# regeirk/pycwt

Measured on NVIDIA H100. Metric: cwt_scale_points_per_sec, higher is better.
Workload: dtype f64

## Files before the change

### pycwt_b200/csrc/engine.cu

```cuda
#include <algorithm>
#include <array>
#include <cmath>
#include <cstdint>
#include <cstdio>
#include <cstdlib>
#include <cstring>
#include <map>
#include <mutex>
#include <set>
#include <string>
#include <type_traits>
#include <vector>

#include <cuda_runtime.h>
#ifndef CWTB_HOST_EMU
#include <dlfcn.h>
#endif

#include "../../include/cwt_b200.h"
#include "kernels.cuh"

using namespace cwtb;

template <class B, class = void> struct BodyNT { static constexpr int value = NT; };
// ... 101 lines not shown
  unsigned n = 0, L = 0;
  double2 *wm = nullptr;
  double2 *bf[2] = {nullptr, nullptr};
};

struct NTabDev {
  double2 *hi = nullptr, *lo = nullptr;
  int h = 0;
};

struct cwtb_ctx {
  int device = 0;
  rt_stream stream{};
  rt_stream aux_stream{};
  rt_stream prio_stream{};
  rt_stream prio_aux[7]{};
  int prio_fan = 4;
  int prio_mode = 1;
  rt_stream chain_streams[3]{};
  int n_chains = 2;
  rt_stream cur{};
  int pad_pow2 = 1;
  int coh_precision = 0;
  std::map<unsigned, BluePlan> blue;
  long long serial = 0;
  int two_streams = 1;
  int three_streams = 1;
  rt_stream copy_streams[4]{};
  int d2h_split = 1;
  std::string err;
  double band_eps = 1e-16;
  double band_eps32 = 1e-9;
  double expand_eps = 5e-13;
  double expand_eps32 = 2e-7;
  int expand_mma = 1;
  int dense_margin = 2;
  int expand_min_log2R = 0;
  int os_on = 1;
  Buf osH, osgrp;
  Buf *ztmp = nullptr;
  void *comm = nullptr;
  int comm_world = 1, comm_rank = 0;
  Buf comm_send, comm_recv;
  int group = 0;
  size_t group_bytes = (size_t)512 << 20;
  size_t rows_chunk_bytes = (size_t)256 << 20;
  int l2_persist = 0;
  int direct_max_log2 = 13;
  int fused = 0;
  int ring = 3;
  int pipe_ahead = 2;
  int num_sms = 132;
  int pf_dist = 132;
  int gauss_rec = 1;
  int pf_rows_a = 32, pf_rows_b = 32;
  int pf_dist_a = 132;
  int k2_512_max_log2 = 16;
  int passb_rev = 1;
  int k2_band_log2 = 9;
  size_t batch_bytes = (size_t)4 << 30;
  double2 *tw64 = nullptr;
  float2 *tw32 = nullptr;
  std::map<unsigned, NTabDev> ntabs;
  Buf filt;
  int filt_rows = 0;
  long long filt_n = 0;
  Buf Zxs[7];
  Buf Zx, Cin, Cout, wtab;
  std::map<std::array<long long, 3>, long long> wtab_index;
  std::vector<double> wtab_host;
  size_t wtab_uploaded = 0;
  size_t wtab_max_bytes = (size_t)256 << 20;
  Buf ctr, sig, sig2, spec, Z, Zc[3], Y, B, W, W2, descs, table, scratch, C, A12, F, aux, rowd, win, mask, hist, noise, wide, blueA, blueX, blueY;
  Job job;
  struct PlanKey {
    long long n0 = -1;
    double dt = 0, param = 0, band_eps = 0, band_eps32 = 0, expand_eps = 0, expand_eps32 = 0;
    int S = 0, family = 0, precision = 0, nbatch = 0, pad = 0;
    std::vector<double> scales;
    bool operator==(const PlanKey &o) const {
      return n0 == o.n0 && dt == o.dt && param == o.param && band_eps == o.band_eps && band_eps32 == o.band_eps32 &&
             expand_eps == o.expand_eps && expand_eps32 == o.expand_eps32 && S == o.S && family == o.family &&
             precision == o.precision && nbatch == o.nbatch && pad == o.pad && scales == o.scales;
// ... 12 lines not shown
  const void *job_dsig = nullptr;
  double last_ms = 0;
  int launches = 0;
  std::set<const void *> configured;
  bool profiling = false;
  int prof_saved_streams = 1;
  const char *prof_tag = "";
  struct ProfRec { std::string name; unsigned gx, gy; int ev; };
  std::vector<ProfRec> prof;
#ifndef CWTB_HOST_EMU
  std::vector<cudaEvent_t> prof_events;
#endif
  std::set<void *> pinned, devallocs;
#ifndef CWTB_HOST_EMU
  cudaEvent_t e0{}, e1{};
  cudaEvent_t ev_fork{}, ev_join{}, ev_joinc[3]{}, ev_coarse{};
  cudaEvent_t ev_h2d[2]{}, ev_used[2]{};
  cudaEvent_t ev_xband{}, ev_pj[7]{}, ev_angle{};
#endif
};

static int fail(cwtb_ctx *c, int code, const std::string &msg);
static void apply_l2_policy(cwtb_ctx *c);
static int fail(cwtb_ctx *c, int code, const std::string &msg) {
  if (c) c->err = msg;
  return code;
}
#define RT(call)                                                                             \
  do {                                                                                       \
    int e_ = (call);                                                                         \
    if (e_ != 0) return fail(c, CWTB_ERR_CUDA, std::string(#call) + ": " + rt_errstr(e_));   \
  } while (0)

// ... 353 lines not shown
    if (xeps > 0 && !job.exact && family != CWTB_TABLE && khi >= klo && job.log2N >= 9 && band_limited) {
      const long long kc = (klo + khi) / 2 - (((klo + khi) % 2 != 0 && (klo + khi) < 0) ? 1 : 0);
      const long long hw = std::max(khi - kc, kc - klo);
#ifdef CWTB_HOST_EMU
      const bool mma = false;
      const int max_taps = precision == CWTB_F64 ? 20 : 10;
#else
      const bool mma = precision == CWTB_F64 && c->expand_mma && job.log2N >= 12;
      const int max_taps = mma ? 20 : (precision == CWTB_F64 ? 16 : 10);
#endif
      const long long need = max_taps > 16 ? (32 * hw + 10) / 11 : 4 * hw;
      int lmin = std::max(6, ilog2((unsigned long long)std::max<long long>(need, 1)));
      lmin = std::max(lmin, job.log2N - 14);
      double best = 1e300;
      const int min_log2R = c->expand_min_log2R ? c->expand_min_log2R : (mma ? 2 : 3);
      for (int l = lmin; l <= lmin + 2 && job.log2N - l >= min_log2R; ++l) {
        double xi_b = 0;
        int w = expand_taps((double)hw / (double)(1ll << l), xeps, precision != CWTB_F64, max_taps, &xi_b);
        if (!w) continue;
        if (mma) w = (w + 3) / 4 * 4;
        if (xi_b > 0.25 && expand_gain(fam, s, klo, khi, kc, l, w, M_PI * w * (1.0 - xi_b)) > 64.0) continue;
        const int ksteps = job.log2N - l == 2 ? (w + 4) / 4 : (w + 3) / 4;
        const double xcost = mma ? std::max(2.72, 0.83 * ksteps) : 0.06 * (2 * w + 8);
        const double cost = xcost + (mma ? 18.0 : 12.0) * (double)(1ll << l) / (double)N;
        if (cost < best) {
          best = cost;
          d.ip_log2Nc = l; d.ip_kc = (int)kc; d.ip_w = w;
          d.ip_beta = M_PI * w * (1.0 - xi_b);
          d.ip_dc = std::cyl_bessel_i(0.0, d.ip_beta) / w;
        }
      }
// ... 106 lines not shown
    case 10: return launch_passA<T, SIGN, 1024, MODE>(c, a, ny);
  }
  return fail(c, CWTB_ERR_UNSUPPORTED, "transform longer than 2^20 per row is not supported yet");
}

template <typename T, int SIGN>
static int two_kernel_rows(cwtb_ctx *c, const void *in, int real_in, long long in_pitch, long long n_in,
                           cx<T> *out, long long out_pitch, unsigned n, int nrows, long long nout,
                           const double *grow, double post, int ileave, const ScaleDesc *descs, int first,
                           int out_row0, int epi) {
  const int l2 = ilog2(n);
  NTab nt;
  int e = get_ntab(c, n, l2, &nt);
  if (e) return e;
  const int chunk = std::max(1, std::min(nrows, (int)std::max<size_t>(1, c->rows_chunk_bytes / ((size_t)n * sizeof(cx<T>)))));
  Buf &Zt = c->ztmp ? *c->ztmp : c->Z;
  if ((e = ensure(c, Zt, (size_t)chunk * n * sizeof(cx<T>)))) return e;
  for (int r0 = 0; r0 < nrows; r0 += chunk) {
    const int nr = std::min(chunk, nrows - r0);
    PassAArgs<T> a{};
    a.in = in; a.Z = (cx<T> *)Zt.p; a.tw = Tw<T>::get(c); a.nt = nt;
    a.in_pitch = in_pitch; a.n_in = n_in; a.N = n; a.first = 0; a.zmod = 1 << 30; a.K2 = K2C;
    a.row0 = (ileave > 1 ? 0 : out_row0) + r0;
    a.pf_dist = c->pf_rows_a;
    e = real_in ? dispatch_passA<T, SIGN, MODE_REAL>(c, l2 - 10, a, nr)
                : dispatch_passA<T, SIGN, MODE_CPLX>(c, l2 - 10, a, nr);
    if (e) return e;
    PassBArgs<T> b{};
    b.Z = (const cx<T> *)Zt.p; b.out = out; b.tw = Tw<T>::get(c); b.descs = descs;
    b.pitch = out_pitch; b.nout = nout; b.N = n; b.first = first;
    b.epi = grow ? EPI_GAUSS : epi; b.grow = grow; b.post = post; b.zmod = 1 << 30;
// ... 496 lines not shown
      cudaEvent_t e;
      RT(cudaEventCreate(&e));
      c->prof_events.push_back(e);
    }
    c->prof.push_back({std::string(c->prof_tag) + body_name(__PRETTY_FUNCTION__), grid, rows, ev});
    RT(cudaEventRecord(c->prof_events[ev], c->cur));
  }
  kern<<<grid, Body::NTB, Body::SMEM, c->cur>>>(a, gm, (unsigned)total);
  RT(cudaGetLastError());
  if (ev >= 0) RT(cudaEventRecord(c->prof_events[ev + 1], c->cur));
  c->launches++;
  return 0;
}
#endif

template <typename T, int TAPS>
static int launch_expand_t(cwtb_ctx *c, const ExpandArgs<T> &a, int rows, int min_log2Nc) {
  using B = ExpandBody<T, TAPS>;
  const unsigned gx = std::max<unsigned>(1, a.N / (unsigned)(B::NT * B::L));
#ifndef CWTB_HOST_EMU
  if constexpr (std::is_same<T, double>::value) {
    static_assert(ExpandMmaBody<TAPS>::OUT_PER_CTA == 4096, "the planner assumes the tensor-core kernel from Np = 2^12");
    if (c->expand_mma && a.N >= (unsigned)ExpandMmaBody<TAPS>::OUT_PER_CTA) {
      const unsigned gm = a.N / (32u * std::min<unsigned>(ExpandMmaBody<TAPS>::L, 1u << min_log2Nc));
      if (a.epi == EPI_MULCONJ) return launch_persistent<ExpandMmaBody<TAPS, EPI_MULCONJ>>(c, gm, rows, a);
      return launch_persistent<ExpandMmaBody<TAPS>>(c, gm, rows, a);
    }
  }
#endif
#ifndef CWTB_HOST_EMU
// ... 24 lines not shown
    }
  }
  return fail(c, CWTB_ERR_STATE, "expansion: unsupported tap count");
}

template <typename T>
static int run_job(cwtb_ctx *c, const Job &job, const T *dsig, cx<T> *Wout = nullptr, int epi = EPI_STORE) {
  using V = cx<T>;
  if (job.exact) {
    if constexpr (std::is_same<T, double>::value) return run_job_exact(c, job, dsig, Wout, epi);
    else return fail(c, CWTB_ERR_UNSUPPORTED, "un-padded transforms run in fp64");
  }
  const unsigned N = job.N;
  const int S = job.S * job.nbatch;
  int e;
  struct CurGuard { cwtb_ctx *c; ~CurGuard() { c->cur = c->stream; c->prof_tag = ""; c->ztmp = nullptr; } } cur_guard{c};
  if ((e = ensure(c, c->spec, (size_t)job.nbatch * N * sizeof(V)))) return e;
  if (!Wout) {
    if ((e = ensure(c, c->W, (size_t)S * job.n0 * sizeof(V)))) return e;
    Wout = (V *)c->W.p;
  }
  V *spec = (V *)c->spec.p;
  V *W = Wout;
  const ScaleDesc *ddesc = (const ScaleDesc *)c->descs.p;
  Fam fam = job.fam;
  if (fam.family == CWTB_TABLE) fam.table = (const double2 *)c->table.p;

  if (N < 32) {
    if (job.nbatch != 1) return fail(c, CWTB_ERR_UNSUPPORTED, "batched transform needs n0 > 16");
    TinyFwdArgs<T> fa{dsig, spec, job.n0, N};
    if ((e = launch<TinyFwdBody<T>>(c, 1, 1, fa))) return e;
// ... 28 lines not shown
    }
  }
  const bool split = c->two_streams != 0;
#ifndef CWTB_HOST_EMU
  const bool split2 = split && c->three_streams && !c->fused;
  if (split) {
    RT(cudaEventRecord(c->ev_fork, c->stream));
    RT(cudaStreamWaitEvent(c->aux_stream, c->ev_fork, 0));
    if (split2)
      for (int k = 1; k < c->n_chains; ++k) RT(cudaStreamWaitEvent(c->chain_streams[k - 1], c->ev_fork, 0));
  }
#else
  const bool split2 = false;
#endif
  if (job.coarse_elems) {
#ifndef CWTB_HOST_EMU
    const bool prio = split && c->prio_mode > 0;
    if (prio) RT(cudaStreamWaitEvent(c->prio_stream, c->ev_fork, 0));
    if (split) c->cur = prio ? c->prio_stream : c->aux_stream;
#endif
    if ((e = ensure(c, c->Cin, job.coarse_elems * sizeof(V)))) return e;
    if ((e = ensure(c, c->Cout, job.coarse_elems * sizeof(V)))) return e;
    int first = -1, maxl = 0, nrows = 0;
    for (const ClassRun &cl : job.classes)
      if (cl.expand) {
        if (first < 0) first = cl.first;
        maxl = std::max(maxl, cl.log2Nc);
        nrows += cl.count;
      }
    ExpandBandArgs<T> xa{ddesc, spec, (V *)c->Cin.p, fam, N, first};
    constexpr int XPER = ExpandBandBody<T>::PER;
    if ((e = launch<ExpandBandBody<T>>(c, ((1u << maxl) + NT * XPER - 1) / (NT * XPER), nrows, xa))) return e;
    c->ztmp = &c->Zx;
    c->prof_tag = "coarse:";
#ifndef CWTB_HOST_EMU
    const int fan = prio ? c->prio_fan : 1;
    int fan_used = 1, group = 0;
    if (fan > 1) RT(cudaEventRecord(c->ev_xband, c->prio_stream));
#endif
    for (size_t ci = 0; ci < job.classes.size() && !e; ++ci) {
      const ClassRun &cl = job.classes[ci];
      if (!cl.expand) continue;
      if (ci == 0 || !job.classes[ci - 1].expand || job.classes[ci - 1].log2Nc != cl.log2Nc) {
        int rows = 0;
        for (size_t cj = ci; cj < job.classes.size() && job.classes[cj].expand && job.classes[cj].log2Nc == cl.log2Nc; ++cj)
          rows += job.classes[cj].count;
        const long long off = job.descs[cl.first].ip_coff;
        const unsigned Nc = 1u << cl.log2Nc;
#ifndef CWTB_HOST_EMU
        if (fan > 1) {
          const int slot = group++ % fan;
          if (slot > 0) {
            if (slot >= fan_used) {
              RT(cudaStreamWaitEvent(c->prio_aux[slot - 1], c->ev_xband, 0));
              fan_used = slot + 1;
            }
            c->cur = c->prio_aux[slot - 1];
            c->ztmp = &c->Zxs[slot - 1];
          } else {
            c->cur = c->prio_stream;
            c->ztmp = &c->Zx;
          }
        }
#endif
        e = fft_rows<T, +1>(c, (const V *)c->Cin.p + off, 0, Nc, Nc, (V *)c->Cout.p + off, Nc, Nc, rows);
      }
    }
#ifndef CWTB_HOST_EMU
    if (fan > 1) {
      for (int k = 1; k < fan_used; ++k) {
        RT(cudaEventRecord(c->ev_pj[k - 1], c->prio_aux[k - 1]));
        RT(cudaStreamWaitEvent(c->prio_stream, c->ev_pj[k - 1], 0));
      }
      c->cur = c->prio_stream;
      c->ztmp = &c->Zx;
    }
#endif
    c->prof_tag = "";
#ifndef CWTB_HOST_EMU
    if (prio && c->prio_mode == 1) {
      RT(cudaEventRecord(c->ev_coarse, c->prio_stream));
      RT(cudaStreamWaitEvent(c->aux_stream, c->ev_coarse, 0));
      c->cur = c->aux_stream;
    }
#endif
    for (size_t ci = 0; ci < job.classes.size() && !e; ++ci) {
      const ClassRun &cl = job.classes[ci];
      if (!cl.expand || (ci > 0 && job.classes[ci - 1].expand && job.classes[ci - 1].taps == cl.taps)) continue;
      int rows = 0, minl = 30;
      for (size_t cj = ci; cj < job.classes.size() && job.classes[cj].expand && job.classes[cj].taps == cl.taps; ++cj) {
        rows += job.classes[cj].count;
        minl = std::min(minl, job.classes[cj].log2Nc);
      }
      ExpandArgs<T> ea{ddesc, (const V *)c->Cout.p, (const double *)c->wtab.p, W, nt, job.n0, N, cl.first, epi,
                       job.log2N};
      e = launch_expand<T>(c, cl.taps, ea, rows, minl);
    }
    c->ztmp = nullptr;
#ifndef CWTB_HOST_EMU
    if (prio && c->prio_mode == 2 && !e) {
      RT(cudaEventRecord(c->ev_coarse, c->prio_stream));
      RT(cudaStreamWaitEvent(c->aux_stream, c->ev_coarse, 0));
    }
#endif
    c->cur = c->stream;
    if (e) return e;
  }
  if (!job.os_groups.empty()) {
    if constexpr (std::is_same<T, double>::value) {
      unsigned gx = 0;
      for (const OsGroup &g : job.os_groups)
        gx = std::max<unsigned>(gx, (unsigned)((job.n0 + (long long)g.hop * OsBody<4>::P - 1) /
                                               ((long long)g.hop * OsBody<4>::P)));
      OsArgs oa{ddesc, (const OsGroup *)c->osgrp.p, dsig, (const double2 *)c->osH.p, W, Tw<T>::get(c),
                job.n0, N, epi};
      if ((e = launch<OsBody<4>>(c, gx, (unsigned)job.os_groups.size(), oa))) return e;
// ... 205 lines not shown
  if (!out) return CWTB_ERR_ARG;
  *out = nullptr;
  cwtb_ctx *c = new cwtb_ctx();
  c->device = device;
#ifndef CWTB_HOST_EMU
  if (cudaSetDevice(device) != cudaSuccess) { delete c; return CWTB_ERR_CUDA; }
  if (cudaStreamCreateWithFlags(&c->stream, cudaStreamNonBlocking) != cudaSuccess) { delete c; return CWTB_ERR_CUDA; }
  cudaEventCreate(&c->e0);
  cudaEventCreate(&c->e1);
  for (auto &st : c->copy_streams) cudaStreamCreateWithFlags(&st, cudaStreamNonBlocking);
  cudaStreamCreateWithFlags(&c->aux_stream, cudaStreamNonBlocking);
  {
    int lo = 0, hi = 0;
    cudaDeviceGetStreamPriorityRange(&lo, &hi);
    cudaStreamCreateWithPriority(&c->prio_stream, cudaStreamNonBlocking, hi);
    for (auto &st : c->prio_aux) cudaStreamCreateWithPriority(&st, cudaStreamNonBlocking, hi);
  }
  cudaEventCreateWithFlags(&c->ev_xband, cudaEventDisableTiming);
  cudaEventCreateWithFlags(&c->ev_angle, cudaEventDisableTiming);
  for (auto &ev : c->ev_pj) cudaEventCreateWithFlags(&ev, cudaEventDisableTiming);
  if (const char *g = getenv("CWTB_PRIO_FAN")) c->prio_fan = std::min(8, std::max(1, atoi(g)));
  cudaEventCreateWithFlags(&c->ev_coarse, cudaEventDisableTiming);
  for (auto &ev : c->ev_h2d) cudaEventCreateWithFlags(&ev, cudaEventDisableTiming);
  for (auto &ev : c->ev_used) cudaEventCreateWithFlags(&ev, cudaEventDisableTiming);
  if (const char *g = getenv("CWTB_BATCH_PIPELINE")) c->batch_pipeline = atoi(g) != 0;
  if (const char *g = getenv("CWTB_PRIO")) c->prio_mode = std::min(2, std::max(0, atoi(g)));
  for (auto &st : c->chain_streams) cudaStreamCreateWithFlags(&st, cudaStreamNonBlocking);
  for (auto &ev : c->ev_joinc) cudaEventCreateWithFlags(&ev, cudaEventDisableTiming);
  cudaEventCreateWithFlags(&c->ev_fork, cudaEventDisableTiming);
  cudaEventCreateWithFlags(&c->ev_join, cudaEventDisableTiming);
  if (const char *g = getenv("CWTB_STREAMS")) { c->two_streams = atoi(g) >= 2; c->three_streams = atoi(g) >= 3; }
  if (const char *g = getenv("CWTB_D2H_SPLIT")) c->d2h_split = std::min(4, std::max(1, atoi(g)));
#endif
  c->cur = c->stream;
  if (const char *g = getenv("CWTB_GROUP")) c->group = std::max(0, atoi(g));
  if (const char *g = getenv("CWTB_GROUP_MB")) c->group_bytes = (size_t)std::max(1, atoi(g)) << 20;
  if (const char *g = getenv("CWTB_ROWS_CHUNK_MB")) c->rows_chunk_bytes = (size_t)std::max(1, atoi(g)) << 20;
// ... 29 lines not shown
  if (const char *g = getenv("CWTB_DIRECT_MAX")) c->direct_max_log2 = std::min(13, std::max(10, atoi(g)));
  int e = init_tables(c);
  if (e == 0) e = rt_sync(c->stream) ? CWTB_ERR_CUDA : 0;
  if (e) { delete c; return e; }
  *out = c;
  return CWTB_OK;
}

void cwtb_destroy(cwtb_ctx *c) {
  if (!c) return;
#ifndef CWTB_HOST_EMU
  cudaSetDevice(c->device);
  cudaStreamSynchronize(c->stream);
#endif
  cwtb_comm_destroy(c);
  for (Buf *b : {&c->osH, &c->osgrp, &c->Zxs[0],&c->Zxs[1], &c->Zxs[2], &c->Zxs[3], &c->Zxs[4], &c->Zxs[5], &c->Zxs[6], &c->stage_dev[0], &c->stage_dev[1], &c->batch_power, &c->filt, &c->comm_send, &c->comm_recv, &c->Zx, &c->Cin, &c->Cout, &c->wtab, &c->ctr, &c->sig, &c->sig2, &c->spec, &c->Z, &c->Zc[0], &c->Zc[1], &c->Zc[2], &c->Y, &c->B, &c->W, &c->W2, &c->descs, &c->table, &c->scratch,
                 &c->C, &c->A12, &c->F, &c->aux, &c->rowd, &c->win, &c->mask, &c->hist, &c->noise, &c->wide, &c->blueA, &c->blueX, &c->blueY, &c->coh})
    if (b->p) rt_free(b->p);
  for (auto &kv : c->ntabs) { rt_free(kv.second.hi); rt_free(kv.second.lo); }
  for (auto &kv : c->blue) { rt_free(kv.second.wm); rt_free(kv.second.bf[0]); rt_free(kv.second.bf[1]); }
  if (c->tw64) rt_free(c->tw64);
  if (c->tw32) rt_free(c->tw32);
  for (void *p : c->pinned) rt_host_free(p);
  for (void *p : c->devallocs) rt_free(p);
#ifndef CWTB_HOST_EMU
  cudaEventDestroy(c->e0);
  cudaEventDestroy(c->e1);
  cudaStreamDestroy(c->stream);
  for (auto &st : c->copy_streams) cudaStreamDestroy(st);
  cudaStreamDestroy(c->aux_stream);
  cudaStreamDestroy(c->prio_stream);
  for (auto &st : c->prio_aux) cudaStreamDestroy(st);
  cudaEventDestroy(c->ev_xband);
  cudaEventDestroy(c->ev_angle);
  for (auto &ev : c->ev_pj) cudaEventDestroy(ev);
  cudaEventDestroy(c->ev_coarse);
  for (auto &ev : c->ev_h2d) cudaEventDestroy(ev);
  for (auto &ev : c->ev_used) cudaEventDestroy(ev);
  for (void *p : c->stage_host) if (p) cudaFreeHost(p);
  for (auto &st : c->chain_streams) cudaStreamDestroy(st);
  for (auto &ev : c->ev_joinc) cudaEventDestroy(ev);
  cudaEventDestroy(c->ev_fork);
  cudaEventDestroy(c->ev_join);
#endif
  delete c;
}

const char *cwtb_last_error(cwtb_ctx *c) { return c ? c->err.c_str() : "null context"; }

int cwtb_set_band_eps(cwtb_ctx *c, double eps) {
  if (!c || !(eps >= 0) || eps >= 1e-6) return fail(c, CWTB_ERR_ARG, "band eps must be in [0, 1e-6)");
// ... 1511 lines not shown
```

### pycwt_b200/csrc/kernels.cuh

```cuda
#pragma once
#include <math.h>
#include "fft_tile.cuh"

namespace cwtb {

struct ScaleDesc {
  double s;
  double amp;
  int row;
  int k_lo, k_hi;
  int log2K;
  int rsplit;
  int trow;
  int chan;
  int pad_;
  long long boff;
  int ip_log2Nc;
  int ip_kc;
  int ip_w;
  int os_grp;
  long long ip_coff;
  long long ip_woff;
  double ip_beta;
  double ip_dc;
// ... 549 lines not shown
      const long long s = a.lo + bx * chunk, e = s + chunk < a.hi ? s + chunk : a.hi;
      double m = 0;
      for (long long i = s + tid; i < e; i += NT) {
        const double2 v = a.h[(size_t)by * a.pitch + i];
        m = fmax(m, fmax(fabs(v.x), fabs(v.y)));
      }
      sm[tid] = m;
    } else if (tid == 0) {
      double m = 0;
      for (int i = 0; i < NT; ++i) m = fmax(m, sm[i]);
      a.out[(size_t)by * a.nblk + bx] = m;
    }
  }
};

enum { MODE_DENSE = 0, MODE_BAND = 1, MODE_REAL = 2, MODE_CPLX = 3 };

template <typename T> struct PassAArgs {
  const ScaleDesc *descs;
  const cx<T> *spec;
  const cx<T> *Bbuf;
  const void *in;
  cx<T> *Z;
  const cx<T> *tw;
  Fam fam;
  NTab nt;
  long long in_pitch, n_in;
  unsigned N;
  int first, row0;
  int zmod;
  int pf_dist;
  int gauss_rec;
  unsigned K2;
};

template <typename T, int K1, int MODE, int SIGN> struct PassABody {
  static constexpr int NTB = TileCfg<T>::NT;
  static constexpr int NT = NTB;
  using V = cx<T>;
  using Args = PassAArgs<T>;
  using LY = Lay<T, K1>;
  static constexpr int NP = Plan<K1>::NP;
  static constexpr int P = LY::P;
  static constexpr int T2 = P < K2C ? P : K2C;
  static constexpr int NPHASE = NP == 1 ? 1 : NP + 1;
  static constexpr size_t SMEM = LY::BYTES;

  struct Src {
    const Args &a;
    ScaleDesc d;
    int by, p;
    V twist0;
    HD Src(const Args &a_, int by_, int p_) : a(a_), by(by_), p(p_) {
      if (MODE == MODE_DENSE || MODE == MODE_BAND) d = a.descs[a.first + by];
    }
    HD V get(int pos, int r2) const {
      const unsigned r = (unsigned)pos * a.K2 + (unsigned)r2;
      if (MODE == MODE_DENSE) {
        const int k = (int)r - (r >= a.N / 2 ? (int)a.N : 0);
        if (a.fam.family != 3 && (k < d.k_lo || k > d.k_hi)) return mk<T>(0, 0);
        return band_value<T>(a.fam, d, a.spec, r, k, a.N);
      } else if (MODE == MODE_BAND) {
        V v = ldg(&a.Bbuf[d.boff + r]);
        if (p == 0 || NP > 1) return v;
        const int k1 = pos - ((int)r >= d.rsplit ? K1 : 0);
        V w = nroot_t<T>(a.nt, (unsigned)k1 * (unsigned)p * a.K2);
        return cmul(v, w);
      } else if (MODE == MODE_REAL) {
        const T *row = (const T *)a.in + (size_t)(a.row0 + by) * a.in_pitch;
        return mk<T>((long long)r < a.n_in ? ldg(&row[r]) : (T)0, (T)0);
      } else {
        const V *row = (const V *)a.in + (size_t)(a.row0 + by) * a.in_pitch;
        return (long long)r < a.n_in ? ldg(&row[r]) : mk<T>(0, 0);
      }
    }
  };

  template <int PH> HD static void phase(const Args &a, int bx, int by, int tid, void *smraw) {
    V *sm = (V *)smraw;
    const int NTILE2 = (int)(a.K2 / T2);
    const int p = bx / NTILE2;
    const int r20 = (bx % NTILE2) * T2;
// ... 119 lines not shown
        ld.pk2 = (unsigned)p * a.K2;
        tile_first<T, K1, SIGN>(sm, a.tw, ld, tid);
      } else {
        SmemLoader<T, K1> ld;
        ld.sm = sm;
        tile_first<T, K1, SIGN>(sm, a.tw, ld, tid);
      }
    } else if constexpr (PH == 2 && NP == 3) {
      tile_second<T, K1, SIGN>(sm, a.tw, tid);
    } else {
      pass_last<T, K1, SIGN>(sm, st, tid);
    }
  }
};

template <typename T> struct ExpandBandArgs {
  const ScaleDesc *descs;
  const cx<T> *spec;
  cx<T> *Cin;
  Fam fam;
  unsigned N;
  int first;
};
template <typename T> struct ExpandBandBody {
  using V = cx<T>;
  using Args = ExpandBandArgs<T>;
  static constexpr int NPHASE = 1;
  static constexpr size_t SMEM = 0;
  static constexpr int PER = 4;
  template <int PH> HD static void phase(const Args &a, int bx, int by, int tid, void *) {
    const ScaleDesc d = a.descs[a.first + by];
    const int Nc = 1 << d.ip_log2Nc;
    const double pw = 3.14159265358979323846 * (double)d.ip_w;
#pragma unroll
    for (int i = 0; i < PER; ++i) {
      const int r = (bx * PER + i) * NT + tid;
      if (r >= Nc) return;
      const int kp = r < Nc / 2 ? r : r - Nc;
      const int k = d.ip_kc + kp;
      V v = mk<T>(0, 0);
      if (k >= d.k_lo && k <= d.k_hi) {
        const V b = band_value<T>(a.fam, d, a.spec, (unsigned)k & (a.N - 1), k, a.N);
        const double x = pw * ((double)kp / (double)Nc);
        const double z = sqrt(d.ip_beta * d.ip_beta - x * x);
        const double f = d.ip_dc * (z / sinh(z));
        v = mk<T>((T)((double)b.x * f), (T)((double)b.y * f));
      }
      a.Cin[d.ip_coff + r] = v;
    }
  }
};

template <typename T> struct ExpandArgs {
  const ScaleDesc *descs;
  const cx<T> *C;
  const double *wt;
  cx<T> *W;
  NTab nt;
  long long n0;
  unsigned N;
  int first;
  int epi;
  int log2N;
};
// ... 1103 lines not shown
```

Baseline: 102.9 billion.

## Fuse coarse band expansion into segmented multi-class coarse FFT kernels

Removes the separate ExpandBandBody pass and its Cin buffer. Coarse band values are now computed directly inside the first FFT phase through a new MODE_COARSE source. Coarse classes are grouped into segments and launched as a few multi-segment kernels: a short-row kernel for lengths up to 2^10, and segmented PassA/PassB kernels for longer rows. The per-class fan-out across several priority streams is replaced by a single dedicated short stream. This is meant to cut launch count and memory traffic, at the cost of segment-lookup overhead and larger switch-dispatched kernels that may lower occupancy.

```diff
diff --git a/profiles/micro/coarse_ab.py b/profiles/micro/coarse_ab.py
--- /dev/null
+++ b/profiles/micro/coarse_ab.py
@@ -0,0 +1,109 @@
+import os
+import subprocess
+import sys
+
+import numpy as np
+
+ROOT = os.path.dirname(os.path.dirname(os.path.dirname(os.path.abspath(__file__))))
+sys.path.insert(0, ROOT)
+import workloads as wl
+import pycwt_b200 as pycwt
+from pycwt_b200 import _engine
+from pycwt_b200.wavelet import _boxcar_len
+from bench import pin_to_gpu_numa_node
+
+
+def identical(arms, fn):
+    a, b = (fn(e) for e in arms.values())
+    if isinstance(a, tuple):
+        return all(np.array_equal(x, y) for x, y in zip(a, b) if x is not None)
+    return np.array_equal(a, b)
+
+
+def main():
+    args = sys.argv[1:]
+    parent = args[0]
+    new = args[1] if len(args) > 1 and not args[1].isdigit() else os.path.join(ROOT, "pycwt_b200", "libcwtb200.so")
+    rounds = int(args[-1]) if args[-1].isdigit() else 6
+    pin_to_gpu_numa_node(0)
+    print(subprocess.run(["nvidia-smi", "--query-gpu=name,power.limit,clocks.max.sm", "--format=csv"],
+                         capture_output=True, text=True).stdout.strip())
+    c = wl.C2
+    x = wl.config2_signal()
+    sj = wl.config2_scales()
+    arms = {"parent": _engine.Engine(0, lib_path=parent), "new": _engine.Engine(0, lib_path=new)}
+    dev = {}
+    launches = {}
+    for name, eng in arms.items():
+        d = eng.dev_alloc(x.nbytes)
+        eng.h2d(d, x)
+        eng.cwt_dev(d, 0, c["n"], c["dt"], sj, _engine.MORLET, c["f0"], _engine.F64)
+        eng.bench_last(10)
+        launches[name] = eng.last_launch_count()
+        dev[name] = d
+    times = {k: [] for k in arms}
+    for _ in range(rounds):
+        for name, eng in arms.items():
+            times[name].append(eng.bench_last(20))
+    for name, t in times.items():
+        print("%-6s config 2 step %.4f ms (min %.4f, max %.4f) over %d runs of 20 steps, %d launches per step" % (
+            name, float(np.median(t)), min(t), max(t), len(t), launches[name]))
+    print("median difference parent - new: %.4f ms" % (float(np.median(times["parent"])) - float(np.median(times["new"]))))
+    for name, eng in arms.items():
+        print(name + ": serialised kernels of one step")
+        for k in sorted(eng.profile_last(), key=lambda k: -k["ms"]):
+            print("      %-52s %3d x  %7.4f ms  rows %d" % (k["name"], k["launches"], k["ms"], k["rows"]))
+    same = True
+    for r0 in range(0, len(sj), 32):
+
+        rows = []
+        for eng in arms.values():
+            out = np.empty((32, c["n"]), np.complex128)
+            eng._check(eng.lib.cwtb_get_w(eng.h, _engine._ptr(out), 1, r0, 32))
+            rows.append(out)
+        same = same and np.array_equal(rows[0], rows[1])
+    print("config 2 W (fp64, 256 rows): %s" % ("bit-identical" if same else "DIFFERENT"))
+    for name, eng in arms.items():
+        eng.dev_free(dev[name])
+    c3 = wl.C3
+    x3 = wl.config3_signal()
+    for fam, code in (("dog", _engine.DOG), ("paul", _engine.PAUL)):
+        p = c3[fam]
+        s3 = wl.geometric_scales(p["s0"], p["dj"], p["J"])
+        for name, eng in arms.items():
+            d = eng.dev_alloc(x3.nbytes)
+            eng.h2d(d, x3)
+            eng.cwt_dev(d, 1, c3["n"], c3["dt"], s3, code, float(p["m"]), _engine.F32)
+            eng.bench_last(10)
+            launches[name] = eng.last_launch_count()
+            dev[name] = d
+        times = {k: [] for k in arms}
+        for _ in range(rounds):
+            for name, eng in arms.items():
+                times[name].append(eng.bench_last(20))
+        for name, t in times.items():
+            print("%-6s config 3 %-4s step %.4f ms (min %.4f, max %.4f), %d launches per step" % (
+                name, fam, float(np.median(t)), min(t), max(t), launches[name]))
+        for name, eng in arms.items():
+            print("%s: serialised kernels of one config 3 %s step" % (name, fam))
+            for k in sorted(eng.profile_last(), key=lambda k: -k["ms"]):
+                print("      %-52s %3d x  %7.4f ms  rows %d" % (k["name"], k["launches"], k["ms"], k["rows"]))
+            eng.dev_free(dev[name])
+    print("config 3 Paul(4) W (fp32): %s" % ("bit-identical" if identical(
+        arms, lambda e: e.cwt(x3, c3["dt"], s3, _engine.PAUL, float(p["m"]), _engine.F32)) else "DIFFERENT"))
+    c4 = wl.C4
+    y1, y2 = wl.config4_signals()
+    s4 = wl.geometric_scales(c4["s0"], c4["dj"], c4["J"])
+    klen = _boxcar_len(pycwt.Morlet(c4["f0"]), c4["dj"])
+    for prec, pname in ((_engine.F64, "fp64"), (_engine.F32, "fp32")):
+        ok_x = identical(arms, lambda e: e.xwt(y1, y2, c4["dt"], s4, _engine.MORLET, c4["f0"], prec))
+        ok_w = identical(arms, lambda e: e.wct(y1, y2, c4["dt"], c4["dj"], s4, _engine.MORLET, c4["f0"], klen,
+                                               True, prec))
+        print("config 4 %s: xwt %s, wct %s" % (pname, "bit-identical" if ok_x else "DIFFERENT",
+                                               "bit-identical" if ok_w else "DIFFERENT"))
+    for eng in arms.values():
+        eng.close()
+
+
+if __name__ == "__main__":
+    main()
diff --git a/profiles/micro/coarse_timeline.py b/profiles/micro/coarse_timeline.py
--- /dev/null
+++ b/profiles/micro/coarse_timeline.py
@@ -0,0 +1,102 @@
+import json
+import os
+import re
+import subprocess
+import sys
+import tempfile
+
+ROOT = os.path.dirname(os.path.dirname(os.path.dirname(os.path.abspath(__file__))))
+sys.path.insert(0, ROOT)
+import workloads as wl
+from pycwt_b200 import _engine
+
+
+def kind(name):
+    n = name.replace("cwtb::", "")
+    if re.search(r"ExpandBandBody|RowsBody|Coarse", n):
+        return "coarse"
+    if re.search(r"Expand(Mma)?Body", n):
+        return "expand"
+    if "OsBody" in n:
+        return "os"
+    if re.search(r"PassABody<double, \d+, 3, 1>|PassABody<float, \d+, 3, 1>", n):
+        return "coarse"
+    if re.search(r"PassABody<\w+, \d+, 2, -1>|PassBBody<\w+, -1", n):
+        return "fwd"
+    if re.search(r"PassABody|PassBBody|BandBody", n):
+        return "dense"
+    return "other"
+
+
+def main():
+    args = [a for a in sys.argv[1:] if not a.startswith("--")]
+    lib = None
+    if "--lib" in sys.argv:
+        lib = sys.argv[sys.argv.index("--lib") + 1]
+        args = [a for a in args if a != lib]
+    out_dir = args[0] if args else os.path.join(tempfile.gettempdir(), "coarse_timeline")
+    os.makedirs(out_dir, exist_ok=True)
+    import torch
+    from torch.profiler import ProfilerActivity, profile
+    torch.zeros(1, device="cuda")
+    print(subprocess.run(["nvidia-smi", "--query-gpu=name,power.limit,clocks.max.sm", "--format=csv"],
+                         capture_output=True, text=True).stdout.strip())
+    c = wl.C2
+    x = wl.config2_signal()
+    sj = wl.config2_scales()
+    eng = _engine.Engine(0, lib_path=lib)
+    d = eng.dev_alloc(x.nbytes)
+    eng.h2d(d, x)
+    eng.cwt_dev(d, 0, c["n"], c["dt"], sj, _engine.MORLET, c["f0"], _engine.F64)
+    eng.bench_last(10)
+    print("step %.4f ms (bench_last(20), profiler off), %d launches per step"
+          % (eng.bench_last(20), eng.last_launch_count()))
+    eng.sync()
+    with profile(activities=[ProfilerActivity.CUDA]) as prof:
+        eng.bench_last(1)
+        eng.sync()
+    path = os.path.join(out_dir, "coarse_timeline.pt.trace.json")
+    prof.export_chrome_trace(path)
+    eng.dev_free(d)
+    eng.close()
+
+    with open(path) as f:
+        ev = [e for e in json.load(f)["traceEvents"] if e.get("cat") == "kernel"]
+    ev.sort(key=lambda e: e["ts"])
+    t0 = ev[0]["ts"]
+    k = [(kind(e["name"]), e["args"].get("stream"), (e["ts"] - t0) / 1e3, (e["ts"] + e["dur"] - t0) / 1e3,
+          e["name"]) for e in ev]
+    end = max(e for _, _, _, e, _ in k)
+    print("step span in the trace: %.3f ms, %d kernels" % (end, len(k)))
+    coarse_streams = sorted({s for kd, s, _, _, _ in k if kd == "coarse"})
+    for s in sorted({s for _, s, _, _, _ in k}):
+        ks = [r for r in k if r[1] == s]
+        gaps = [b[2] - a[3] for a, b in zip(ks, ks[1:]) if b[2] > a[3]]
+        kinds = {}
+        for r in ks:
+            kinds[r[0]] = kinds.get(r[0], 0) + 1
+        print("stream %-4s %3d kernels %-40s %.3f .. %.3f ms, busy %.3f ms, idle gaps %d totalling %.3f ms "
+              "(largest %.3f)" % (s, len(ks), kinds, ks[0][2], ks[-1][3], sum(r[3] - r[2] for r in ks),
+                                  len(gaps), sum(gaps), max(gaps) if gaps else 0.0))
+        if s in coarse_streams:
+            for r in ks:
+                print("      %-7s %.3f .. %.3f  %s" % (r[0], r[2], r[3], r[4][:110]))
+    co = [r for r in k if r[0] == "coarse"]
+    co += [r for r in k if r[0] == "dense" and r[1] in coarse_streams and "PassBBody" in r[4]]
+    ex = [r for r in k if r[0] == "expand"]
+    if co:
+        print("coarse chain: %d kernels, %.3f .. %.3f ms, %.3f ms of kernel time"
+              % (len(co), min(r[2] for r in co), max(r[3] for r in co), sum(r[3] - r[2] for r in co)))
+    if ex:
+        print("first expansion launch starts at %.3f ms; expansion launches end at %.3f ms"
+              % (min(r[2] for r in ex), max(r[3] for r in ex)))
+    other = [r for r in k if r[0] in ("os", "dense") and r[1] not in coarse_streams]
+
+    def overlap(a, b):
+        return max(0.0, min(a[3], b[3]) - max(a[2], b[2]))
+    print("coarse kernels overlapping overlap-save / dense launches: %.3f ms (sum over pairs)"
+          % sum(overlap(a, b) for a in co for b in other))
+
+
+if __name__ == "__main__":
+    main()
diff --git a/pycwt_b200/csrc/engine.cu b/pycwt_b200/csrc/engine.cu
--- a/pycwt_b200/csrc/engine.cu
+++ b/pycwt_b200/csrc/engine.cu
@@ -139,8 +139,7 @@
   rt_stream stream{};
   rt_stream aux_stream{};
   rt_stream prio_stream{};
-  rt_stream prio_aux[7]{};
-  int prio_fan = 4;
+  rt_stream prio_short{};
   int prio_mode = 1;
   rt_stream chain_streams[3]{};
   int n_chains = 2;
@@ -163,7 +162,6 @@
   int expand_min_log2R = 0;
   int os_on = 1;
   Buf osH, osgrp;
-  Buf *ztmp = nullptr;
   void *comm = nullptr;
   int comm_world = 1, comm_rank = 0;
   Buf comm_send, comm_recv;
@@ -190,8 +188,7 @@
   Buf filt;
   int filt_rows = 0;
   long long filt_n = 0;
-  Buf Zxs[7];
-  Buf Zx, Cin, Cout, wtab;
+  Buf Zx, Cout, wtab;
   std::map<std::array<long long, 3>, long long> wtab_index;
   std::vector<double> wtab_host;
   size_t wtab_uploaded = 0;
@@ -234,9 +231,9 @@
   std::set<void *> pinned, devallocs;
 #ifndef CWTB_HOST_EMU
   cudaEvent_t e0{}, e1{};
-  cudaEvent_t ev_fork{}, ev_join{}, ev_joinc[3]{}, ev_coarse{};
+  cudaEvent_t ev_fork{}, ev_join{}, ev_joinc[3]{}, ev_coarse{}, ev_coarse_short{};
   cudaEvent_t ev_h2d[2]{}, ev_used[2]{};
-  cudaEvent_t ev_xband{}, ev_pj[7]{}, ev_angle{};
+  cudaEvent_t ev_angle{};
 #endif
 };
 
@@ -620,7 +617,7 @@
       lmin = std::max(lmin, job.log2N - 14);
       double best = 1e300;
       const int min_log2R = c->expand_min_log2R ? c->expand_min_log2R : (mma ? 2 : 3);
-      for (int l = lmin; l <= lmin + 2 && job.log2N - l >= min_log2R; ++l) {
+      for (int l = lmin; l <= lmin + 2 && l <= 20 && job.log2N - l >= min_log2R; ++l) {
         double xi_b = 0;
         int w = expand_taps((double)hw / (double)(1ll << l), xeps, precision != CWTB_F64, max_taps, &xi_b);
         if (!w) continue;
@@ -757,7 +754,7 @@
   int e = get_ntab(c, n, l2, &nt);
   if (e) return e;
   const int chunk = std::max(1, std::min(nrows, (int)std::max<size_t>(1, c->rows_chunk_bytes / ((size_t)n * sizeof(cx<T>)))));
-  Buf &Zt = c->ztmp ? *c->ztmp : c->Z;
+  Buf &Zt = c->Z;
   if ((e = ensure(c, Zt, (size_t)chunk * n * sizeof(cx<T>)))) return e;
   for (int r0 = 0; r0 < nrows; r0 += chunk) {
     const int nr = std::min(chunk, nrows - r0);
@@ -1284,6 +1281,22 @@
 }
 #endif
 
+template <class Body, typename T>
+static int launch_coarse(cwtb_ctx *c, CoarseArgs<T> a, const std::vector<CoarseSeg> &segs) {
+  for (size_t s0 = 0; s0 < segs.size(); s0 += CSEG_MAX) {
+    a.nseg = (int)std::min<size_t>(CSEG_MAX, segs.size() - s0);
+    unsigned ctas = 0;
+    for (int i = 0; i < a.nseg; ++i) {
+      a.seg[i] = segs[s0 + i];
+      a.seg[i].cta0 = (int)ctas;
+      ctas += (unsigned)Body::ctas(a.seg[i].log2Nc, a.seg[i].count);
+    }
+    int e = launch<Body>(c, ctas, 1, a);
+    if (e) return e;
+  }
+  return 0;
+}
+
 template <typename T, int TAPS>
 static int launch_expand_t(cwtb_ctx *c, const ExpandArgs<T> &a, int rows, int min_log2Nc) {
   using B = ExpandBody<T, TAPS>;
@@ -1338,7 +1351,7 @@
   const unsigned N = job.N;
   const int S = job.S * job.nbatch;
   int e;
-  struct CurGuard { cwtb_ctx *c; ~CurGuard() { c->cur = c->stream; c->prof_tag = ""; c->ztmp = nullptr; } } cur_guard{c};
+  struct CurGuard { cwtb_ctx *c; ~CurGuard() { c->cur = c->stream; c->prof_tag = ""; } } cur_guard{c};
   if ((e = ensure(c, c->spec, (size_t)job.nbatch * N * sizeof(V)))) return e;
   if (!Wout) {
     if ((e = ensure(c, c->W, (size_t)S * job.n0 * sizeof(V)))) return e;
@@ -1397,92 +1410,77 @@
   const bool split2 = false;
 #endif
   if (job.coarse_elems) {
-#ifndef CWTB_HOST_EMU
     const bool prio = split && c->prio_mode > 0;
-    if (prio) RT(cudaStreamWaitEvent(c->prio_stream, c->ev_fork, 0));
+#ifndef CWTB_HOST_EMU
+    if (prio) {
+      RT(cudaStreamWaitEvent(c->prio_stream, c->ev_fork, 0));
+      RT(cudaStreamWaitEvent(c->prio_short, c->ev_fork, 0));
+    }
     if (split) c->cur = prio ? c->prio_stream : c->aux_stream;
 #endif
-    if ((e = ensure(c, c->Cin, job.coarse_elems * sizeof(V)))) return e;
     if ((e = ensure(c, c->Cout, job.coarse_elems * sizeof(V)))) return e;
-    int first = -1, maxl = 0, nrows = 0;
-    for (const ClassRun &cl : job.classes)
-      if (cl.expand) {
-        if (first < 0) first = cl.first;
-        maxl = std::max(maxl, cl.log2Nc);
-        nrows += cl.count;
-      }
-    ExpandBandArgs<T> xa{ddesc, spec, (V *)c->Cin.p, fam, N, first};
-    constexpr int XPER = ExpandBandBody<T>::PER;
-    if ((e = launch<ExpandBandBody<T>>(c, ((1u << maxl) + NT * XPER - 1) / (NT * XPER), nrows, xa))) return e;
-    c->ztmp = &c->Zx;
-    c->prof_tag = "coarse:";
-#ifndef CWTB_HOST_EMU
-    const int fan = prio ? c->prio_fan : 1;
-    int fan_used = 1, group = 0;
-    if (fan > 1) RT(cudaEventRecord(c->ev_xband, c->prio_stream));
-#endif
-    for (size_t ci = 0; ci < job.classes.size() && !e; ++ci) {
+    std::vector<CoarseSeg> short_segs, long_segs;
+    size_t zx_elems = 0;
+    for (size_t ci = 0; ci < job.classes.size(); ++ci) {
       const ClassRun &cl = job.classes[ci];
       if (!cl.expand) continue;
-      if (ci == 0 || !job.classes[ci - 1].expand || job.classes[ci - 1].log2Nc != cl.log2Nc) {
-        int rows = 0;
-        for (size_t cj = ci; cj < job.classes.size() && job.classes[cj].expand && job.classes[cj].log2Nc == cl.log2Nc; ++cj)
+      if (cl.log2Nc < 6 || cl.log2Nc > 20)
+        return fail(c, CWTB_ERR_STATE, "expansion: coarse length outside 2^6 .. 2^20");
+      std::vector<CoarseSeg> &v = cl.log2Nc <= 10 ? short_segs : long_segs;
+      if (ci > 0 && job.classes[ci - 1].expand && job.classes[ci - 1].log2Nc == cl.log2Nc) v.back().count += cl.count;
+      else v.push_back(CoarseSeg{cl.first, cl.count, cl.log2Nc, 0});
+      if (cl.log2Nc > 10)
+        zx_elems = std::max(zx_elems, (size_t)job.descs[cl.first].ip_coff + ((size_t)cl.count << cl.log2Nc));
+    }
+    CoarseArgs<T> ca{};
+    ca.descs = ddesc; ca.spec = spec; ca.C = (V *)c->Cout.p; ca.tw = Tw<T>::get(c); ca.fam = fam; ca.Nx = N;
+    ca.pf_dist = c->pf_rows_b; ca.rev = c->passb_rev;
+    c->prof_tag = "coarse:";
+    if (!long_segs.empty()) {
+      if ((e = ensure(c, c->Zx, zx_elems * sizeof(V)))) return e;
+      ca.Z = (V *)c->Zx.p;
+      for (const CoarseSeg &g : long_segs)
+        if ((e = get_ntab(c, 1u << g.log2Nc, g.log2Nc, &ca.nt[g.log2Nc - 10]))) return e;
+      if ((e = launch_coarse<CoarseABody<T>>(c, ca, long_segs))) return e;
+      if ((e = launch_coarse<CoarseBBody<T>>(c, ca, long_segs))) return e;
+    }
+    if (!short_segs.empty()) {
+#ifndef CWTB_HOST_EMU
+      if (prio) c->cur = c->prio_short;
+#endif
+      if ((e = launch_coarse<CoarseRowsBody<T>>(c, ca, short_segs))) return e;
+    }
+    c->prof_tag = "";
+#ifndef CWTB_HOST_EMU
+    if (prio) {
+      RT(cudaEventRecord(c->ev_coarse_short, c->prio_short));
+      RT(cudaEventRecord(c->ev_coarse, c->prio_stream));
+      c->cur = c->prio_mode == 1 ? c->aux_stream : c->prio_stream;
+      RT(cudaStreamWaitEvent(c->cur, c->ev_coarse_short, 0));
+    }
+#endif
+    for (int pass = 0; pass < 2 && !e; ++pass) {
+#ifndef CWTB_HOST_EMU
+      if (pass == 1 && prio && c->prio_mode == 1) RT(cudaStreamWaitEvent(c->cur, c->ev_coarse, 0));
+#endif
+      for (size_t ci = 0; ci < job.classes.size() && !e; ++ci) {
+        const ClassRun &cl = job.classes[ci];
+        if (!cl.expand || (ci > 0 && job.classes[ci - 1].expand && job.classes[ci - 1].taps == cl.taps)) continue;
+        int rows = 0, minl = 30, maxl = 0;
+        for (size_t cj = ci; cj < job.classes.size() && job.classes[cj].expand && job.classes[cj].taps == cl.taps; ++cj) {
           rows += job.classes[cj].count;
-        const long long off = job.descs[cl.first].ip_coff;
-        const unsigned Nc = 1u << cl.log2Nc;
-#ifndef CWTB_HOST_EMU
-        if (fan > 1) {
-          const int slot = group++ % fan;
-          if (slot > 0) {
-            if (slot >= fan_used) {
-              RT(cudaStreamWaitEvent(c->prio_aux[slot - 1], c->ev_xband, 0));
-              fan_used = slot + 1;
-            }
-            c->cur = c->prio_aux[slot - 1];
-            c->ztmp = &c->Zxs[slot - 1];
-          } else {
-            c->cur = c->prio_stream;
-            c->ztmp = &c->Zx;
-          }
+          minl = std::min(minl, job.classes[cj].log2Nc);
+          maxl = std::max(maxl, job.classes[cj].log2Nc);
         }
-#endif
-        e = fft_rows<T, +1>(c, (const V *)c->Cin.p + off, 0, Nc, Nc, (V *)c->Cout.p + off, Nc, Nc, rows);
+        if ((maxl > 10) != (pass == 1)) continue;
+        ExpandArgs<T> ea{ddesc, (const V *)c->Cout.p, (const double *)c->wtab.p, W, nt, job.n0, N, cl.first, epi,
+                         job.log2N};
+        e = launch_expand<T>(c, cl.taps, ea, rows, minl);
       }
     }
 #ifndef CWTB_HOST_EMU
-    if (fan > 1) {
-      for (int k = 1; k < fan_used; ++k) {
-        RT(cudaEventRecord(c->ev_pj[k - 1], c->prio_aux[k - 1]));
-        RT(cudaStreamWaitEvent(c->prio_stream, c->ev_pj[k - 1], 0));
-      }
-      c->cur = c->prio_stream;
-      c->ztmp = &c->Zx;
-    }
-#endif
-    c->prof_tag = "";
-#ifndef CWTB_HOST_EMU
-    if (prio && c->prio_mode == 1) {
-      RT(cudaEventRecord(c->ev_coarse, c->prio_stream));
-      RT(cudaStreamWaitEvent(c->aux_stream, c->ev_coarse, 0));
-      c->cur = c->aux_stream;
-    }
-#endif
-    for (size_t ci = 0; ci < job.classes.size() && !e; ++ci) {
-      const ClassRun &cl = job.classes[ci];
-      if (!cl.expand || (ci > 0 && job.classes[ci - 1].expand && job.classes[ci - 1].taps == cl.taps)) continue;
-      int rows = 0, minl = 30;
-      for (size_t cj = ci; cj < job.classes.size() && job.classes[cj].expand && job.classes[cj].taps == cl.taps; ++cj) {
-        rows += job.classes[cj].count;
-        minl = std::min(minl, job.classes[cj].log2Nc);
-      }
-      ExpandArgs<T> ea{ddesc, (const V *)c->Cout.p, (const double *)c->wtab.p, W, nt, job.n0, N, cl.first, epi,
-                       job.log2N};
-      e = launch_expand<T>(c, cl.taps, ea, rows, minl);
-    }
-    c->ztmp = nullptr;
-#ifndef CWTB_HOST_EMU
-    if (prio && c->prio_mode == 2 && !e) {
-      RT(cudaEventRecord(c->ev_coarse, c->prio_stream));
+    if (prio && !e) {
+      if (c->prio_mode == 2) RT(cudaEventRecord(c->ev_coarse, c->prio_stream));
       RT(cudaStreamWaitEvent(c->aux_stream, c->ev_coarse, 0));
     }
 #endif
@@ -1718,13 +1716,11 @@
     int lo = 0, hi = 0;
     cudaDeviceGetStreamPriorityRange(&lo, &hi);
     cudaStreamCreateWithPriority(&c->prio_stream, cudaStreamNonBlocking, hi);
-    for (auto &st : c->prio_aux) cudaStreamCreateWithPriority(&st, cudaStreamNonBlocking, hi);
-  }
-  cudaEventCreateWithFlags(&c->ev_xband, cudaEventDisableTiming);
+    cudaStreamCreateWithPriority(&c->prio_short, cudaStreamNonBlocking, hi);
+  }
   cudaEventCreateWithFlags(&c->ev_angle, cudaEventDisableTiming);
-  for (auto &ev : c->ev_pj) cudaEventCreateWithFlags(&ev, cudaEventDisableTiming);
-  if (const char *g = getenv("CWTB_PRIO_FAN")) c->prio_fan = std::min(8, std::max(1, atoi(g)));
   cudaEventCreateWithFlags(&c->ev_coarse, cudaEventDisableTiming);
+  cudaEventCreateWithFlags(&c->ev_coarse_short, cudaEventDisableTiming);
   for (auto &ev : c->ev_h2d) cudaEventCreateWithFlags(&ev, cudaEventDisableTiming);
   for (auto &ev : c->ev_used) cudaEventCreateWithFlags(&ev, cudaEventDisableTiming);
   if (const char *g = getenv("CWTB_BATCH_PIPELINE")) c->batch_pipeline = atoi(g) != 0;
@@ -1784,7 +1780,7 @@
   cudaStreamSynchronize(c->stream);
 #endif
   cwtb_comm_destroy(c);
-  for (Buf *b : {&c->osH, &c->osgrp, &c->Zxs[0],&c->Zxs[1], &c->Zxs[2], &c->Zxs[3], &c->Zxs[4], &c->Zxs[5], &c->Zxs[6], &c->stage_dev[0], &c->stage_dev[1], &c->batch_power, &c->filt, &c->comm_send, &c->comm_recv, &c->Zx, &c->Cin, &c->Cout, &c->wtab, &c->ctr, &c->sig, &c->sig2, &c->spec, &c->Z, &c->Zc[0], &c->Zc[1], &c->Zc[2], &c->Y, &c->B, &c->W, &c->W2, &c->descs, &c->table, &c->scratch,
+  for (Buf *b : {&c->osH, &c->osgrp, &c->stage_dev[0], &c->stage_dev[1], &c->batch_power, &c->filt, &c->comm_send, &c->comm_recv, &c->Zx, &c->Cout, &c->wtab, &c->ctr, &c->sig, &c->sig2, &c->spec, &c->Z, &c->Zc[0], &c->Zc[1], &c->Zc[2], &c->Y, &c->B, &c->W, &c->W2, &c->descs, &c->table, &c->scratch,
                  &c->C, &c->A12, &c->F, &c->aux, &c->rowd, &c->win, &c->mask, &c->hist, &c->noise, &c->wide, &c->blueA, &c->blueX, &c->blueY, &c->coh})
     if (b->p) rt_free(b->p);
   for (auto &kv : c->ntabs) { rt_free(kv.second.hi); rt_free(kv.second.lo); }
@@ -1800,11 +1796,10 @@
   for (auto &st : c->copy_streams) cudaStreamDestroy(st);
   cudaStreamDestroy(c->aux_stream);
   cudaStreamDestroy(c->prio_stream);
-  for (auto &st : c->prio_aux) cudaStreamDestroy(st);
-  cudaEventDestroy(c->ev_xband);
+  cudaStreamDestroy(c->prio_short);
   cudaEventDestroy(c->ev_angle);
-  for (auto &ev : c->ev_pj) cudaEventDestroy(ev);
   cudaEventDestroy(c->ev_coarse);
+  cudaEventDestroy(c->ev_coarse_short);
   for (auto &ev : c->ev_h2d) cudaEventDestroy(ev);
   for (auto &ev : c->ev_used) cudaEventDestroy(ev);
   for (void *p : c->stage_host) if (p) cudaFreeHost(p);
diff --git a/pycwt_b200/csrc/kernels.cuh b/pycwt_b200/csrc/kernels.cuh
--- a/pycwt_b200/csrc/kernels.cuh
+++ b/pycwt_b200/csrc/kernels.cuh
@@ -587,7 +587,21 @@
   }
 };
 
-enum { MODE_DENSE = 0, MODE_BAND = 1, MODE_REAL = 2, MODE_CPLX = 3 };
+enum { MODE_DENSE = 0, MODE_BAND = 1, MODE_REAL = 2, MODE_CPLX = 3, MODE_COARSE = 4 };
+
+template <typename T> HD cx<T> coarse_value(const Fam &fam, const ScaleDesc &d, const cx<T> *spec, int r, unsigned Nx) {
+  const int Nc = 1 << d.ip_log2Nc;
+  const int kp = r < Nc / 2 ? r : r - Nc;
+  const int k = d.ip_kc + kp;
+  if (k < d.k_lo || k > d.k_hi) return mk<T>(0, 0);
+  const cx<T> b = band_value<T>(fam, d, spec, (unsigned)k & (Nx - 1), k, Nx);
+  const double pw = 3.14159265358979323846 * (double)d.ip_w;
+  const double x = pw * ((double)kp / (double)Nc);
+  const double bb = d.ip_beta * d.ip_beta;
+  const double z = sqrt(fma(-x, x, bb));
+  const double f = d.ip_dc * (z / sinh(z));
+  return mk<T>((T)((double)b.x * f), (T)((double)b.y * f));
+}
 
 template <typename T> struct PassAArgs {
   const ScaleDesc *descs;
@@ -605,6 +619,7 @@
   int pf_dist;
   int gauss_rec;
   unsigned K2;
+  unsigned Nx;
 };
 
 template <typename T, int K1, int MODE, int SIGN> struct PassABody {
@@ -625,7 +640,7 @@
     int by, p;
     V twist0;
     HD Src(const Args &a_, int by_, int p_) : a(a_), by(by_), p(p_) {
-      if (MODE == MODE_DENSE || MODE == MODE_BAND) d = a.descs[a.first + by];
+      if (MODE == MODE_DENSE || MODE == MODE_BAND || MODE == MODE_COARSE) d = a.descs[a.first + by];
     }
     HD V get(int pos, int r2) const {
       const unsigned r = (unsigned)pos * a.K2 + (unsigned)r2;
@@ -639,6 +654,8 @@
         const int k1 = pos - ((int)r >= d.rsplit ? K1 : 0);
         V w = nroot_t<T>(a.nt, (unsigned)k1 * (unsigned)p * a.K2);
         return cmul(v, w);
+      } else if (MODE == MODE_COARSE) {
+        return coarse_value<T>(a.fam, d, a.spec, (int)r, a.Nx);
       } else if (MODE == MODE_REAL) {
         const T *row = (const T *)a.in + (size_t)(a.row0 + by) * a.in_pitch;
         return mk<T>((long long)r < a.n_in ? ldg(&row[r]) : (T)0, (T)0);
@@ -788,40 +805,162 @@
   }
 };
 
-template <typename T> struct ExpandBandArgs {
+struct CoarseSeg { int first, count, log2Nc, cta0; };
+constexpr int CSEG_MAX = 32;
+HD constexpr size_t cmax(size_t a, size_t b) { return a > b ? a : b; }
+template <typename T> struct CoarseArgs {
   const ScaleDesc *descs;
   const cx<T> *spec;
-  cx<T> *Cin;
+  cx<T> *Z;
+  cx<T> *C;
+  const cx<T> *tw;
   Fam fam;
-  unsigned N;
-  int first;
-};
-template <typename T> struct ExpandBandBody {
+  NTab nt[11];
+  unsigned Nx;
+  int nseg;
+  int pf_dist, rev;
+  CoarseSeg seg[CSEG_MAX];
+};
+template <typename T> HD const CoarseSeg &coarse_seg(const CoarseArgs<T> &a, int bx) {
+  int s = 0;
+  while (s + 1 < a.nseg && bx >= a.seg[s + 1].cta0) ++s;
+  return a.seg[s];
+}
+
+template <typename T> struct CoarseRowsBody {
+  static constexpr int NTB = TileCfg<T>::NT;
+  static constexpr int NT = NTB;
   using V = cx<T>;
-  using Args = ExpandBandArgs<T>;
-  static constexpr int NPHASE = 1;
-  static constexpr size_t SMEM = 0;
-  static constexpr int PER = 4;
-  template <int PH> HD static void phase(const Args &a, int bx, int by, int tid, void *) {
-    const ScaleDesc d = a.descs[a.first + by];
-    const int Nc = 1 << d.ip_log2Nc;
-    const double pw = 3.14159265358979323846 * (double)d.ip_w;
-#pragma unroll
-    for (int i = 0; i < PER; ++i) {
-      const int r = (bx * PER + i) * NT + tid;
-      if (r >= Nc) return;
-      const int kp = r < Nc / 2 ? r : r - Nc;
-      const int k = d.ip_kc + kp;
-      V v = mk<T>(0, 0);
-      if (k >= d.k_lo && k <= d.k_hi) {
-        const V b = band_value<T>(a.fam, d, a.spec, (unsigned)k & (a.N - 1), k, a.N);
-        const double x = pw * ((double)kp / (double)Nc);
-        const double z = sqrt(d.ip_beta * d.ip_beta - x * x);
-        const double f = d.ip_dc * (z / sinh(z));
-        v = mk<T>((T)((double)b.x * f), (T)((double)b.y * f));
-      }
-      a.Cin[d.ip_coff + r] = v;
-    }
+  using Args = CoarseArgs<T>;
+  template <int K> static constexpr size_t bytes() { return Lay<T, K>::BYTES; }
+  static constexpr size_t SMEM = cmax(cmax(cmax(bytes<64>(), bytes<128>()), cmax(bytes<256>(), bytes<512>())), bytes<1024>());
+  static constexpr int NPHASE = 4;
+  HD static int ctas(int log2Nc, int rows) {
+    const int P = TileCfg<T>::TILE >> log2Nc;
+    return (rows + P - 1) / P;
+  }
+  struct Storer {
+    V *out;
+    int nb;
+    int K;
+    template <int R> HD void store(int b, int ql, int qs, V (&x)[R]) const {
+      if (b >= nb) return;
+#pragma unroll
+      for (int c = 0; c < R; ++c) out[(size_t)b * K + ql + c * qs] = x[c];
+    }
+  };
+  template <int K, int PH> HD static void tile(const Args &a, const CoarseSeg &g, int bx, int tid, V *sm) {
+    using LY = Lay<T, K>;
+    constexpr int NP = Plan<K>::NP;
+    static_assert(NP >= 2, "coarse rows: multi-pass tile plans only");
+    const int row0 = (bx - g.cta0) * LY::P;
+    const int nb = g.count - row0 < LY::P ? g.count - row0 : LY::P;
+    if constexpr (PH == 0) {
+      for (int idx = tid; idx < LY::P * K; idx += NT) {
+        const int b = idx / K, pos = idx % K;
+        V v = mk<T>(0, 0);
+        if (b < nb) v = coarse_value<T>(a.fam, a.descs[g.first + row0 + b], a.spec, pos, a.Nx);
+        sm[LY::phys(b, pos)] = v;
+      }
+    } else if constexpr (PH == 1) {
+      SmemLoader<T, K> ld;
+      ld.sm = sm;
+      tile_first<T, K, +1>(sm, a.tw, ld, tid);
+    } else if constexpr (PH == 2 && NP == 3) {
+      tile_second<T, K, +1>(sm, a.tw, tid);
+    } else if constexpr (PH == NP) {
+      Storer st{a.C + a.descs[g.first].ip_coff + (size_t)row0 * K, nb, K};
+      pass_last<T, K, +1>(sm, st, tid);
+    }
+  }
+  template <int PH> HD static void phase(const Args &a, int bx, int, int tid, void *smraw) {
+    const CoarseSeg &g = coarse_seg(a, bx);
+    V *sm = (V *)smraw;
+    switch (g.log2Nc) {
+      case 6: tile<64, PH>(a, g, bx, tid, sm); break;
+      case 7: tile<128, PH>(a, g, bx, tid, sm); break;
+      case 8: tile<256, PH>(a, g, bx, tid, sm); break;
+      case 9: tile<512, PH>(a, g, bx, tid, sm); break;
+      case 10: tile<1024, PH>(a, g, bx, tid, sm); break;
+    }
+  }
+};
+
+template <typename T> struct CoarseABody {
+  static constexpr int NTB = TileCfg<T>::NT;
+  static constexpr int NT = NTB;
+  using V = cx<T>;
+  using Args = CoarseArgs<T>;
+  template <int K1> using A = PassABody<T, K1, MODE_COARSE, +1>;
+  static constexpr size_t SMEM = cmax(cmax(cmax(cmax(A<2>::SMEM, A<4>::SMEM), cmax(A<8>::SMEM, A<16>::SMEM)),
+                                           cmax(cmax(A<32>::SMEM, A<64>::SMEM), cmax(A<128>::SMEM, A<256>::SMEM))),
+                                      cmax(A<512>::SMEM, A<1024>::SMEM));
+  static constexpr int NPHASE = 4;
+  template <int K1> HD static int per_row() { return K2C / A<K1>::T2; }
+  HD static int ctas(int log2Nc, int rows) {
+    switch (log2Nc - 10) {
+      case 1: return rows * per_row<2>();
+      case 2: return rows * per_row<4>();
+      case 3: return rows * per_row<8>();
+      case 4: return rows * per_row<16>();
+      case 5: return rows * per_row<32>();
+      case 6: return rows * per_row<64>();
+      case 7: return rows * per_row<128>();
+      case 8: return rows * per_row<256>();
+      case 9: return rows * per_row<512>();
+      case 10: return rows * per_row<1024>();
+    }
+    return 0;
+  }
+  template <int K1, int PH> HD static void tile(const Args &a, const CoarseSeg &g, int bx, int tid, void *sm) {
+    if constexpr (PH < A<K1>::NPHASE) {
+      const int local = bx - g.cta0, per = per_row<K1>();
+      PassAArgs<T> pa{};
+      pa.descs = a.descs; pa.spec = a.spec; pa.tw = a.tw; pa.fam = a.fam; pa.nt = a.nt[g.log2Nc - 10];
+      pa.Z = a.Z + a.descs[g.first].ip_coff;
+      pa.N = 1u << g.log2Nc; pa.Nx = a.Nx; pa.first = g.first; pa.zmod = 1 << 30; pa.K2 = K2C;
+      A<K1>::template phase<PH>(pa, local % per, local / per, tid, sm);
+    }
+  }
+  template <int PH> HD static void phase(const Args &a, int bx, int, int tid, void *sm) {
+    const CoarseSeg &g = coarse_seg(a, bx);
+    switch (g.log2Nc - 10) {
+      case 1: tile<2, PH>(a, g, bx, tid, sm); break;
+      case 2: tile<4, PH>(a, g, bx, tid, sm); break;
+      case 3: tile<8, PH>(a, g, bx, tid, sm); break;
+      case 4: tile<16, PH>(a, g, bx, tid, sm); break;
+      case 5: tile<32, PH>(a, g, bx, tid, sm); break;
+      case 6: tile<64, PH>(a, g, bx, tid, sm); break;
+      case 7: tile<128, PH>(a, g, bx, tid, sm); break;
+      case 8: tile<256, PH>(a, g, bx, tid, sm); break;
+      case 9: tile<512, PH>(a, g, bx, tid, sm); break;
+      case 10: tile<1024, PH>(a, g, bx, tid, sm); break;
+    }
+  }
+};
+
+template <typename T> struct CoarseBBody {
+  using B = PassBBody<T, +1>;
+  static constexpr int NTB = B::NTB;
+  static constexpr int NT = NTB;
+  using Args = CoarseArgs<T>;
+  static constexpr size_t SMEM = B::SMEM;
+  static constexpr int NPHASE = B::NPHASE;
+  HD static int per_row(int log2Nc) {
+    constexpr int P = B::LY::P;
+    return ((1 << (log2Nc - 10)) + P - 1) / P;
+  }
+  HD static int ctas(int log2Nc, int rows) { return rows * per_row(log2Nc); }
+  template <int PH> HD static void phase(const Args &a, int bx, int, int tid, void *sm) {
+    const CoarseSeg &g = coarse_seg(a, bx);
+    const int local = bx - g.cta0, per = per_row(g.log2Nc);
+    const long long off = a.descs[g.first].ip_coff;
+    const unsigned Nc = 1u << g.log2Nc;
+    PassBArgs<T> pb{};
+    pb.Z = a.Z + off; pb.out = a.C + off; pb.tw = a.tw;
+    pb.pitch = Nc; pb.nout = Nc; pb.N = Nc; pb.post = 1.0;
+    pb.epi = EPI_STORE; pb.zmod = 1 << 30; pb.pf_dist = a.pf_dist; pb.ny = g.count; pb.ileave = 1; pb.rev = a.rev;
+    B::template phase<PH>(pb, local % per, local / per, tid, sm);
   }
 };
 
```

Measured after the change: 107.1 billion, median of 6. +4.1%, better.
